# Sangluisme/PSgradientSDF

Measured on AMD Instinct MI355X. Metric: Gauss-Newton iterations/sec (full PS sweep), 256^3 grid x 50 frames, higher is better.
Workload: dtype f32

## Files before the change

psgradientsdf_amd/capi.py:

```python
from __future__ import annotations

import ctypes as C
import os

import numpy as np

ALBEDO, LIGHT, DIST, POSE, ALL = 1, 2, 4, 8, 15
SH1, SH2, LED = 0, 1, 2
L2, CAUCHY, HUBER, TUKEY, TRUNC_L2 = 0, 1, 2, 3, 4
R_DEPTH, R_NORMAL, R_ALBEDO, R_SHADING, R_RENDERED, R_RESIDUAL, R_VOXEL = 1, 2, 4, 8, 16, 32, 64
R_ALL = 127
_R_PLANES = [("depth", R_DEPTH, 1), ("normal", R_NORMAL, 3), ("albedo", R_ALBEDO, 3), ("shading", R_SHADING, 1),
             ("rendered", R_RENDERED, 3), ("residual", R_RESIDUAL, 3), ("voxel", R_VOXEL, 1)]

_HERE = os.path.dirname(os.path.abspath(__file__))
ENGINE_LIB = os.environ.get("PSGSDF_ENGINE_LIB") or os.path.join(_HERE, "csrc", "libpsgsdf.so")
ENGINE_LIB_DEV = os.path.join(_HERE, "csrc", "libpsgsdf_dev.so")


class GridDesc(C.Structure):
    _fields_ = [("dim", C.c_int32 * 3), ("voxel_size", C.c_float), ("shift", C.c_float * 3), ("truncation", C.c_float)]


class Settings(C.Structure):
# ... 806 lines not shown
                    cross_rank_ready=out[4] % 10, halo_pushes=out[4] // 10, cross_rank_solves=out[5], cross_rank_mem_kind=out[6], probe_stale=out[7] // 1000000, probe_timeouts=out[7] % 1000000)

    def debug_rare_rows(self):
        r = C.c_int64(); w = C.c_int64()
        self._check(self._fn("debug_rare_rows")(self.ctx, C.byref(r), C.byref(w)), "debug_rare_rows")
        return r.value, w.value

    def debug_frame_system(self, block):
        i = self.info()
        if block == LIGHT:
            n = i.light_stride; nb = 1 if self._settings.model == LED else i.n_frames
        else:
            n = 6; nb = i.n_frames
        H = np.empty((nb, n, n), np.float64); b = np.empty((nb, n), np.float64)
        self._check(self._fn("debug_frame_system")(self.ctx, C.c_int(block), H.ctypes.data_as(C.c_void_p), b.ctypes.data_as(C.c_void_p)), "debug_frame_system")
        return H, b

    def set_frame_solver(self, mode):
        self._check(self._fn("set_frame_solver")(self.ctx, C.c_int(mode)), "set_frame_solver")

    def frame_solver_stats(self, block):
        it = C.c_int32(); err = C.c_double(); ok = C.c_int32(); ap = C.c_int32()
        self._check(self._fn("get_frame_solver_stats")(self.ctx, C.c_int(block), C.byref(it), C.byref(err), C.byref(ok), C.byref(ap)), "get_frame_solver_stats")
        return {"cg_iters": it.value, "cg_error": err.value, "cg_converged": ok.value, "applied": ap.value}

    def debug_frame_cg(self, H, b, max_it=0):
        H = np.ascontiguousarray(H, np.float32); b = np.ascontiguousarray(b, np.float32)
        nb, n = b.shape
        x = np.empty((nb, n), np.float32); it = C.c_int32(); err = C.c_double(); ok = C.c_int32()
        self._check(self._fn("debug_frame_cg")(self.ctx, C.c_int(nb), C.c_int(n), H.ctypes.data_as(C.c_void_p), b.ctypes.data_as(C.c_void_p), x.ctypes.data_as(C.c_void_p),
                                               C.c_int(max_it), C.byref(it), C.byref(err), C.byref(ok)), "debug_frame_cg")
        return x, it.value, err.value, bool(ok.value)

    def debug_albedo_system(self):
        S = self.info().n_band
        H = np.empty((S, 3), np.float32); b = np.empty((S, 3), np.float32)
        self._check(self._fn("debug_albedo_system")(self.ctx, H.ctypes.data_as(C.c_void_p), b.ctypes.data_as(C.c_void_p)), "debug_albedo_system")
        return H, b


class CommXfer(C.Structure):
    _fields_ = [("ptr_dev", C.c_void_p), ("bytes", C.c_size_t), ("peer", C.c_int)]


ALLREDUCE_FN = C.CFUNCTYPE(C.c_int, C.c_void_p, C.c_void_p, C.c_int, C.c_void_p)
SENDRECV_FN = C.CFUNCTYPE(C.c_int, C.c_void_p, C.POINTER(CommXfer), C.c_int, C.POINTER(CommXfer), C.c_int, C.c_void_p)


class CommOps(C.Structure):
    _fields_ = [("user", C.c_void_p), ("allreduce_f64", ALLREDUCE_FN), ("sendrecv", SENDRECV_FN)]


def comm_unique_id() -> bytes:
    buf = (C.c_uint8 * 128)()
    f = engine_lib().psgsdf_comm_unique_id; f.restype = C.c_int
    rc = f(buf)
    if rc != 0:
        raise PsgsdfError(f"psgsdf_comm_unique_id failed rc={rc} (librccl could not be loaded?)")
    return bytes(buf)


def grid_of(sc) -> GridDesc:
    g = GridDesc()
    g.dim[:] = [int(x) for x in sc.dim]
    g.voxel_size = float(sc.voxel_size)
    g.shift[:] = [float(x) for x in sc.shift]
# ... 20 lines not shown
```

psgradientsdf_amd/csrc/api_debug.hip:

```cpp
#include "engine_internal.h"

using namespace psge;

extern "C" {
int psgsdf_set_profiling(psgsdf_ctx* c, int enabled) { if (!c) return PSGSDF_ERR_ARG; c->profiling = enabled != 0; return PSGSDF_OK; }
int psgsdf_reset_kernel_times(psgsdf_ctx* c) { if (!c) return PSGSDF_ERR_ARG; c->ktimes.clear(); c->watch_used = 0; return PSGSDF_OK; }
int psgsdf_watch_kernel(psgsdf_ctx* c, const char* name) {
    if (!c) return PSGSDF_ERR_ARG;
    hipStreamSynchronize(c->stream);
    std::string w = name ? name : ""; int every = 1;
    const size_t sl = w.find('/');
    if (sl != std::string::npos) { every = std::max(1, atoi(w.c_str() + sl + 1)); w.resize(sl); }
    c->watch = w; c->watch_every = every; c->watch_seen = 0; c->watch_used = 0;
    return PSGSDF_OK;
}
int psgsdf_kernel_times(psgsdf_ctx* c, const char** names, double* ms, int64_t* launches, int cap) {
    if (!c) return 0;
    if (c->watch_used) {
        hipStreamSynchronize(c->stream);
        KTime& k = c->ktimes[c->watch];
        for (size_t i = 0; i < c->watch_used; ++i) { float t = 0; if (hipEventElapsedTime(&t, c->watch_pool[i].first, c->watch_pool[i].second) == hipSuccess) { k.ms += t; k.n += 1; } }
        c->watch_used = 0;
    }
    int n = 0;
    for (auto& kv : c->ktimes) { if (n >= cap) break; names[n] = kv.first.c_str(); ms[n] = kv.second.ms; launches[n] = kv.second.n; ++n; }
    return n;
}

int psgsdf_debug_dist_system(psgsdf_ctx* c, float* diag, float* rhs, const float* x, float* y) {
    if (!c || !c->inited) return fail(c, PSGSDF_ERR_STATE, "init first");
    HIPCHK(c, hipSetDevice(c->device));
    SweepArgs a = make_args(c, c->reg_l != 0.f);
    launch_sweep_dist(a, c->stream);
// ... 131 lines not shown
int psgsdf_get_frame_solver_stats(psgsdf_ctx* c, int block, int32_t* iterations, double* error, int32_t* converged, int32_t* applied) {
    if (!c) return PSGSDF_ERR_ARG;
    if (block != PSGSDF_LIGHT && block != PSGSDF_POSE) return fail(c, PSGSDF_ERR_ARG, "block must be LIGHT or POSE");
    HIPCHK(c, hipSetDevice(c->device));
    const int kind = block == PSGSDF_POSE ? 1 : 0;
    psgsdf_step_stats st; memset(&st, 0, sizeof(st));
    if (int rc = read_frame_solver_stats(c, kind, &st)) return rc;
    if (iterations) *iterations = st.cg_iters;
    if (error) *error = st.cg_error;
    if (converged) *converged = st.cg_converged;
    if (applied) *applied = st.applied;
    return PSGSDF_OK;
}
int psgsdf_debug_frame_cg(psgsdf_ctx* c, int nb, int n, const float* H, const float* b, float* x, int max_it, int32_t* iterations, double* error, int32_t* converged) {
    if (!c || !H || !b || !x || nb <= 0) return fail(c, PSGSDF_ERR_ARG, "null argument");
    if ((n != 3 && n != 4 && n != 6 && n != 9) || (long long)nb * n > 2048) return fail(c, PSGSDF_ERR_UNSUPPORTED, "block size %d x %d blocks", n, nb);
    HIPCHK(c, hipSetDevice(c->device));
    float *dH = nullptr, *db = nullptr, *dx = nullptr; double* ds = nullptr;
    const size_t nH = (size_t)nb * n * n, nv = (size_t)nb * n;
    int rc = PSGSDF_OK;
    if (hipMalloc(&dH, sizeof(float) * nH) != hipSuccess || hipMalloc(&db, sizeof(float) * nv) != hipSuccess || hipMalloc(&dx, sizeof(float) * nv) != hipSuccess || hipMalloc(&ds, sizeof(double) * 4) != hipSuccess)
        rc = fail(c, PSGSDF_ERR_DEVICE, "out of device memory");
    double st[4] = {0, 0, 0, 0};
    if (!rc && (hipMemcpy(dH, H, sizeof(float) * nH, hipMemcpyHostToDevice) != hipSuccess || hipMemcpy(db, b, sizeof(float) * nv, hipMemcpyHostToDevice) != hipSuccess)) rc = fail(c, PSGSDF_ERR_DEVICE, "upload failed");
    if (!rc && launch_frames_eigen_raw(nb, n, dH, db, dx, ds, max_it, c->stream)) rc = fail(c, PSGSDF_ERR_UNSUPPORTED, "shape");
    if (!rc && (hipStreamSynchronize(c->stream) != hipSuccess || hipMemcpy(x, dx, sizeof(float) * nv, hipMemcpyDeviceToHost) != hipSuccess || hipMemcpy(st, ds, sizeof(st), hipMemcpyDeviceToHost) != hipSuccess))
        rc = fail(c, PSGSDF_ERR_DEVICE, "%s", hipGetErrorString(hipGetLastError()));
    hipFree(dH); hipFree(db); hipFree(dx); hipFree(ds);
    if (rc) return rc;
    if (iterations) *iterations = (int32_t)st[0];
    if (error) *error = st[1];
    if (converged) *converged = (int32_t)st[2];
    return PSGSDF_OK;
}
int psgsdf_debug_frame_system(psgsdf_ctx* c, int block, double* H, double* b) {
    if (!c || !c->inited || !H || !b) return fail(c, PSGSDF_ERR_STATE, "init first");
    HIPCHK(c, hipSetDevice(c->device));
    SweepArgs a = make_args(c, 0);
    const bool led = c->set.model == PSGSDF_LED;
    int n, nb, nh;
    int launched = 0;
    if (block == PSGSDF_LIGHT) { launched = launch_sweep_light(a, c->stream); n = led ? 3 : (c->set.model == PSGSDF_SH2 ? 9 : 4); nb = led ? 1 : c->F; nh = led ? 3 : n * (n + 1) / 2; }
    else if (block == PSGSDF_POSE) { launched = launch_sweep_pose(a, c->stream); n = 6; nb = c->F; nh = 21; }
    else return fail(c, PSGSDF_ERR_ARG, "block must be LIGHT or POSE");
    if (!launched) HIPCHK(c, hipMemsetAsync(c->acc_frame, 0, sizeof(double) * c->acc_frame_n, c->stream));
    std::vector<double> acc(c->acc_frame_n);
    HIPCHK(c, hipMemcpyAsync(acc.data(), c->acc_frame, sizeof(double) * c->acc_frame_n, hipMemcpyDeviceToHost, c->stream));
    HIPCHK(c, hipStreamSynchronize(c->stream));
    if (led && block == PSGSDF_LIGHT) {
        for (int i = 0; i < 9; ++i) H[i] = 0;
        for (int i = 0; i < 3; ++i) { b[i] = 0; for (int f = 0; f < c->F; ++f) { H[i * 3 + i] += acc[(size_t)f * kFrameRow + i]; b[i] += acc[(size_t)f * kFrameRow + 3 + i]; } }
        return PSGSDF_OK;
    }
    for (int k = 0; k < nb; ++k) {
        const double* A = acc.data() + (size_t)k * kFrameRow;
        double* Hk = H + (size_t)k * n * n; double* bk = b + (size_t)k * n;
        for (int i = 0; i < n * n; ++i) Hk[i] = 0;
        int q = 0;
        for (int i = 0; i < n; ++i) for (int j = i; j < n; ++j) { Hk[i * n + j] = A[q]; Hk[j * n + i] = A[q]; ++q; }
        for (int i = 0; i < n; ++i) bk[i] = A[nh + i];
    }
    return PSGSDF_OK;
}

int psgsdf_debug_albedo_system(psgsdf_ctx* c, float* H, float* b) {
    if (!c || !c->inited || !H || !b) return fail(c, PSGSDF_ERR_STATE, "init first");
// ... 68 lines not shown
```

psgradientsdf_amd/csrc/engine.h:

```cpp
#pragma once
#include <hip/hip_runtime.h>
#include <stdint.h>

namespace psg {

constexpr int kBlock = 256;
constexpr int kMaxFramesLds = 640;
constexpr int kNQ = 19;
constexpr int kNQCommon = 13;
constexpr int kMaxBasis = 9;

struct FrameP {
    float R[9];
    float t[3];
    float l[9];
    float pad[3];
};

struct Cam { float fx, fy, cx, cy; int W, H; };

struct GridP {
    int dim[3];
    long long nvox;
    float vs, vs_inv;
// ... 134 lines not shown
void launch_select_vis(const uint64_t* vis_seq, int wpv_seq, uint64_t* vis_key, int KW, const int* frame_idx, int F, long long nvox, hipStream_t s);
void launch_band_flags(const float* dist, const uint64_t* vis_key, int KW, float vs, long long nvox, int* flags, hipStream_t s);
void launch_band_scan(int* flags_inout_rowof, long long nvox, int* block_sums, int* d_total, hipStream_t s);
struct DenseView { float* dist; float* g[3]; float* weight; float* rho[3]; uint64_t* vis; int KW; int* row_of; };
void launch_band_fill(const DenseView& d, const GridP& grid, Band b, int* d_reach, hipStream_t s);
void launch_band_scatter(const DenseView& d, Band b, hipStream_t s);
void launch_derive(const SweepArgs& a, int update_grad, hipStream_t s);
constexpr int kObsChunk = 2048;
void launch_obs_count(const Band& b, int F, int row0, int row1, int* counts, hipStream_t s);
void launch_block_work(const Band& b, int row0, int row1, int* work, hipStream_t s);
void launch_obs_fill(const Band& b, int F, int row0, int row1, const int* offsets, hipStream_t s);
void launch_lower_bound(const int* lin, int S, int target, int* out, hipStream_t s);
struct SlotList { int n; int id[8]; };
void launch_sum_parts(const double* part, int PB, int nblk, const SlotList& slots, double* out, unsigned long long key, hipStream_t s, const XfTable* xf = nullptr, long long xf_epoch = 0);
void launch_frame_cols(const double* frame, int F, int col, double* out, unsigned long long key, hipStream_t s);
void launch_zero_f64(double* p, int n, hipStream_t s);
struct CopySegs { int n; unsigned off[16]; unsigned len[16]; unsigned long long key[16]; };
void launch_copy_segs(const double* src, double* dst, const CopySegs& segs, hipStream_t s);
void launch_marker(double* p, double v, hipStream_t s);
void launch_init_albedo(const SweepArgs& a, hipStream_t s);
void launch_led_light_init(const SweepArgs& a, hipStream_t s);
void launch_energy(const SweepArgs& a, hipStream_t s);
void launch_sweep_albedo(const SweepArgs& a, hipStream_t s);
void launch_apply_albedo(const SweepArgs& a, hipStream_t s);
void launch_restore_albedo(const SweepArgs& a, hipStream_t s);
int launch_sweep_light(const SweepArgs& a, hipStream_t s);
int launch_sweep_pose(const SweepArgs& a, hipStream_t s);
void launch_solve_light(const SweepArgs& a, FrameP* frames, float* led_light, double* e_out, unsigned long long e_key, float* undo, hipStream_t s);
void launch_restore_light(int F, FrameP* frames, float* led_light, const float* undo, hipStream_t s);
void launch_solve_pose(const SweepArgs& a, FrameP* frames, double* e_out, unsigned long long e_key, hipStream_t s);
bool frames_eigen_fits(int model, int F);
void launch_frames_eigen_light(const SweepArgs& a, FrameP* frames, float* led_light, double* e_out, unsigned long long e_key, float* undo, double* stats, hipStream_t s);
void launch_frames_eigen_pose(const SweepArgs& a, FrameP* frames, double* e_out, unsigned long long e_key, double* stats, hipStream_t s);
int launch_frames_eigen_raw(int nb, int n, const float* H, const float* b, float* x, double* stats, int max_it, hipStream_t s);
void launch_sweep_dist(const SweepArgs& a, hipStream_t s);
void launch_assemble(const SweepArgs& a, hipStream_t s);
void launch_cgf_init(const SweepArgs& a, double* fs, double* part, int G, hipStream_t s);
void launch_cgf_pass(const SweepArgs& a, double* fs, double* part, int G, int rows, int k, int kmax, double* mb, hipStream_t s, int ablate = 0);
void launch_cgf_sum(double* part, int G, int k, double* out, hipStream_t s);
constexpr int kSolveGranPlanes = 8;
constexpr int kSolveThreadsHost = 512, kSolveMaxBlocksHost = 256, kSolveMaxRowsHost = 4, kSolveMbSlots = 24;
int cgf_solve_max_blocks(int rows);
void launch_solve_windows(const Band& b, int row0, int row1, int G, int rows_per_wg, int* tab , int* max_total, hipStream_t s);
int cgf_solve_window_budget(int rows_per_wg);
int launch_cgf_solve(const SweepArgs& a, double* fs, double* gran, int G, int rows_per_wg, int kmax, double* mb, unsigned long long mb_key, int force_passes, hipStream_t s, const XrArgs* xr = nullptr);
void launch_areg_tables(const DenseView& d, const GridP& g, const SweepArgs& a, hipStream_t s);
void launch_areg_build(const SweepArgs& a, hipStream_t s);
void launch_areg_system(const SweepArgs& a, hipStream_t s);
void launch_areg_jx(const SweepArgs& a, const float* p, float* t, hipStream_t s);
void launch_areg_jt(const SweepArgs& a, const float* p, const float* t, float* q, hipStream_t s);
void launch_areg_cg_init(const SweepArgs& a, hipStream_t s);
void launch_areg_cg_iteration(const SweepArgs& a, int i, int nblk, float thr, hipStream_t s);
void launch_areg_cg_update(const SweepArgs& a, float alpha, hipStream_t s);
void launch_areg_cg_dir(const SweepArgs& a, float beta, hipStream_t s);
void launch_apply_albedo_delta(const SweepArgs& a, const float* delta, hipStream_t s);
void launch_matvec(const SweepArgs& a, const float* x, float* y, hipStream_t s);
void launch_apply_dist(const SweepArgs& a, hipStream_t s);
void launch_upsample(const DenseView& src, const DenseView& dst, const GridP& g_old, hipStream_t s);
void launch_fill_f32(float* p, float v, long long n, hipStream_t s);
void launch_normals(const float* depth, const float* cache, int W, int H, int r, double* tmp, float* out, hipStream_t s);
void launch_track(const DenseView& d, const GridP& g, const Cam& cam, const FrameP& fp, const float* depth, float z_min, float z_max, double* part, int nblk, int gdimz, int zown0, int zown1, hipStream_t s);
void launch_integrate(const DenseView& d, uint64_t* vis_seq, int wpv_seq, const GridP& g, const Cam& cam, const FrameP& fp,
                      const float* rgb, const float* depth, const float* normals, int counter, float z_min, float z_max, hipStream_t s);

constexpr int kRenderBrick = 8;
constexpr int kRenderTile = 8;
// ... 73 lines not shown
```

psgradientsdf_amd/csrc/sweeps.hip:

```cpp
#include "device_common.h"

#ifndef PSG_FM_PIPE
#define PSG_FM_PIPE 3
#endif
#ifndef PSG_POSE_WAVES
#define PSG_POSE_WAVES 1
#endif

namespace psg {

__global__ void __launch_bounds__(kBlock) k_init_albedo(SweepArgs a) {
#pragma clang fp contract(off)
    FrameP* sf = reinterpret_cast<FrameP*>(psg_dyn_smem);
    load_frames(sf, a.frames, a.F);
    const Band& b = a.b;
    int j = a.row0 + blockIdx.x * blockDim.x + threadIdx.x;
    if (j >= a.row1) return;
    const float4 p0 = b.vp[0][j];
    float xs[3] = {p0.x, p0.y, p0.z};
    int count = 0; float rho[3] = {0, 0, 0};
    FOR_EACH_VISIBLE_FRAME(b, j, a.F, f) {
        Proj pr = project(xs, frame_at(sf, f), a.cam);
        if (!pr.ok) continue;
        float I[3];
        sample<false>(a.im, f, a.cam, pr.m, pr.n, I, nullptr, nullptr);
        rho[0] += I[0]; rho[1] += I[1]; rho[2] += I[2]; count++;
    }
    if (count) {
#pragma unroll
        for (int k = 0; k < 3; ++k) set_rho(b, j, k, rho[k] / (float)count);
    }
}
void launch_init_albedo(const SweepArgs& a, hipStream_t s) {
    if (a.row1 > a.row0) hipLaunchKernelGGL(k_init_albedo, dim3((a.row1 - a.row0 + kBlock - 1) / kBlock), dim3(kBlock), a.F * sizeof(FrameP), s, a);
}

template <int MODEL, int LOSS, int IMG, bool LED_INIT = false>
__global__ void __launch_bounds__(kBlock) k_energy(SweepArgs a) {
    { __shared__ double fred[kBlock / 64]; fold_pending(a, fred); }
// ... 133 lines not shown
    if (j >= a.row1) return;
#pragma unroll
    for (int ch = 0; ch < 3; ++ch) set_rho(b, j, ch, b.aH[(size_t)ch * b.Spad + j]);
}
void launch_restore_albedo(const SweepArgs& a, hipStream_t s) {
    if (a.row1 > a.row0) hipLaunchKernelGGL(k_restore_albedo, dim3((a.row1 - a.row0 + kBlock - 1) / kBlock), dim3(kBlock), 0, s, a);
}
void launch_apply_albedo(const SweepArgs& a, hipStream_t s) {
    if (a.row1 > a.row0) hipLaunchKernelGGL(k_apply_albedo, dim3((a.row1 - a.row0 + kBlock - 1) / kBlock), dim3(kBlock), 0, s, a);
}

static int fm_rows(const SweepArgs& a, int slots_per_cu) {
    if (const char* e = getenv("PSGSDF_FM_ROWS")) { int v = atoi(e); if (v >= 4 && v <= 64) return v; }
    const long long total = a.b.obs_ptr_total > 0 ? a.b.obs_ptr_total : (long long)a.b.obs_max * a.F;
    const long long slots = 256LL * slots_per_cu;
    long long r = (total + (long long)(0.92 * slots) * kBlock - 1) / ((long long)(0.92 * slots) * kBlock);
    return (int)std::min<long long>(std::max<long long>(r, 4), 64);
}

template <int N> __device__ void solve_spd(const double* Hin, const double* bin, double* x);

__device__ __forceinline__ double ldrow(const double* p) { return __hip_atomic_load(p, __ATOMIC_RELAXED, __HIP_MEMORY_SCOPE_AGENT); }
template <int NB>
__device__ __forceinline__ void frame_solve_light_sh(FrameP* frames, int f, const double* acc, float* undo) {
    constexpr int NH = NB * (NB + 1) / 2;
    if (undo) for (int i = 0; i < 9; ++i) undo[f * 9 + i] = frames[f].l[i];
    double Hd[NB * NB], bd[NB], xd[NB];
    int q = 0;
    for (int i = 0; i < NB; ++i) for (int k = i; k < NB; ++k) { double v = (double)(float)ldrow(acc + q++); Hd[i * NB + k] = v; Hd[k * NB + i] = v; }
    for (int i = 0; i < NB; ++i) bd[i] = (double)(float)ldrow(acc + NH + i);
    solve_spd<NB>(Hd, bd, xd);
    for (int i = 0; i < NB; ++i) frames[f].l[i] -= (float)xd[i];
}
__device__ __forceinline__ void frame_solve_pose(const SweepArgs& a, FrameP* frames, int f, const double* acc) {
    double Hd[36], bd[6], xd[6];
    int q = 0;
    for (int i = 0; i < 6; ++i) for (int k = i; k < 6; ++k) {
        float v = (float)ldrow(acc + q++);
        if (i == k && a.damping != 0.0f) v += a.damping * v;
        Hd[i * 6 + k] = (double)v; Hd[k * 6 + i] = (double)v;
    }
    for (int i = 0; i < 6; ++i) bd[i] = (double)(float)ldrow(acc + 21 + i);
    solve_spd<6>(Hd, bd, xd);
    float xi[6];
    for (int i = 0; i < 6; ++i) xi[i] = (float)xd[i];
    pose_update(frames, f, xi);
}

template <int NV, int KIND, int MODEL>
__device__ __forceinline__ void frame_tail(const SweepArgs& a, double* lds, bool solve_all) {
    if (solve_all) {
        for (int ff = threadIdx.x; ff < a.F; ff += blockDim.x) {
            const double* row = a.acc.frame + (size_t)ff * kFrameRow;
            if (KIND == 0) { if (!ModelTraits<MODEL>::LED) frame_solve_light_sh<ModelTraits<MODEL>::NB == 3 ? 4 : ModelTraits<MODEL>::NB>(a.fm_frames, ff, row, a.fm_undo); }
            else frame_solve_pose(a, a.fm_frames, ff, row);
        }
        __syncthreads();
    }
    if (KIND == 0 && ModelTraits<MODEL>::LED) {
        constexpr int NHL = 3;
        __shared__ float s_dl[3];
        if (a.fm_undo) {
            for (int i = threadIdx.x; i < a.F * 9; i += blockDim.x) a.fm_undo[i] = a.fm_frames[i / 9].l[i % 9];
            if (threadIdx.x < 3) a.fm_undo[a.F * 9 + threadIdx.x] = a.fm_led_light[threadIdx.x];
        }
        __shared__ double srow[6 * kMaxFramesLds];
        for (int i = threadIdx.x; i < 6 * a.F; i += blockDim.x) { const int ff = i / 6, c6 = i % 6; srow[c6 * kMaxFramesLds + ff] = __hip_atomic_load(a.acc.frame + (size_t)ff * kFrameRow + (c6 < 3 ? c6 : NHL + c6 - 3), __ATOMIC_RELAXED, __HIP_MEMORY_SCOPE_AGENT); }
        __syncthreads();
        if (threadIdx.x < 3) {
            const int ch = threadIdx.x;
            double hs = 0, bs = 0;
            for (int ff = 0; ff < a.F; ++ff) { hs += srow[ch * kMaxFramesLds + ff]; bs += srow[(3 + ch) * kMaxFramesLds + ff]; }
            float h = (float)hs; const float bb = (float)bs;
            if (a.damping != 0.0f) h += a.damping * h;
            double Hd[1] = {(double)h}, bd[1] = {(double)bb}, xd[1];
            solve_spd<1>(Hd, bd, xd);
            s_dl[ch] = (float)xd[0];
        }
        __syncthreads();
        for (int ff = threadIdx.x; ff < a.F; ff += blockDim.x) {
#pragma unroll
            for (int ch = 0; ch < 3; ++ch) { const float nl = a.fm_frames[ff].l[ch] - s_dl[ch]; a.fm_frames[ff].l[ch] = nl; if (ff == 0) a.fm_led_light[ch] = nl; }
        }
    }
    if (a.fm_e_out) {
        constexpr int col_e = NV - 2;
        double e = 0, n = 0;
        for (int ff = threadIdx.x; ff < a.F; ff += blockDim.x) {
            e += __hip_atomic_load(a.acc.frame + (size_t)ff * kFrameRow + col_e, __ATOMIC_RELAXED, __HIP_MEMORY_SCOPE_AGENT);
            n += __hip_atomic_load(a.acc.frame + (size_t)ff * kFrameRow + col_e + 1, __ATOMIC_RELAXED, __HIP_MEMORY_SCOPE_AGENT);
        }
        e = wave_sum(e); n = wave_sum(n);
        const int lane = threadIdx.x & 63, w = threadIdx.x >> 6;
        __syncthreads();
        if (lane == 0) { lds[2 * w] = e; lds[2 * w + 1] = n; }
        __syncthreads();
        if (threadIdx.x == 0) { double te = 0, tn = 0; for (int i = 0; i < (int)(blockDim.x >> 6); ++i) { te += lds[2 * i]; tn += lds[2 * i + 1]; } mbox_put(a.fm_e_out, 2, 0, te, a.fm_e_key); mbox_put(a.fm_e_out, 2, 1, tn, a.fm_e_key); mbox_commit(a.fm_e_key); }
    }
}

template <int NV, int KIND, int MODEL>
__device__ __forceinline__ void frame_rows_publish(const SweepArgs& a, int cx, int f, double* lds ) {
    __shared__ int s_last;
    double* dst = a.acc.fpart + ((size_t)f * a.acc.fcap + cx) * kFrameRow;
    if (threadIdx.x < NV) {
        double s = 0;
        for (int i = 0; i < kBlock / 64; ++i) s += lds[i * NV + threadIdx.x];
        __hip_atomic_store(dst + threadIdx.x, s, __ATOMIC_RELAXED, __HIP_MEMORY_SCOPE_AGENT);
    }
    if (threadIdx.x < 64) {
        asm volatile("s_waitcnt vmcnt(0)" ::: "memory");
        if (threadIdx.x == 0) s_last = __hip_atomic_fetch_add(a.acc.fdone + f, 1, __ATOMIC_RELAXED, __HIP_MEMORY_SCOPE_AGENT) == (int)gridDim.x - 1;
    }
    __syncthreads();
    if (!s_last) return;
    if (threadIdx.x == 0) __hip_atomic_store(a.acc.fdone + f, 0, __ATOMIC_RELAXED, __HIP_MEMORY_SCOPE_AGENT);
    const bool solve = a.fm_solve != 0;
    if (threadIdx.x < NV) {
        const double* p = a.acc.fpart + (size_t)f * a.acc.fcap * kFrameRow + threadIdx.x;
        double s = 0;
        for (int c = 0; c < (int)gridDim.x; c += 16) {
            double v[16];
#pragma unroll
            for (int j = 0; j < 16; ++j) v[j] = c + j < (int)gridDim.x ? __hip_atomic_load(p + (size_t)(c + j) * kFrameRow, __ATOMIC_RELAXED, __HIP_MEMORY_SCOPE_AGENT) : 0.0;
#pragma unroll
            for (int j = 0; j < 16; ++j) s += v[j];
        }
        if (solve && a.xf) {
            const XfTable& t = *a.xf;
            const int Rk = t.n_ranks, buf = (int)(a.xf_epoch & 1);
            const long long slot = ((long long)buf * Rk + t.rank) * t.F + f;
            for (int r = 0; r < Rk; ++r) store8_system(t.region[r] + t.pay + slot * kFrameRow + threadIdx.x, s);
            asm volatile("s_waitcnt vmcnt(0)" ::: "memory");
            if (threadIdx.x == 0) for (int r = 0; r < Rk; ++r) __hip_atomic_store(t.region[r] + t.flg + slot, (double)a.xf_epoch, __ATOMIC_RELAXED, __HIP_MEMORY_SCOPE_SYSTEM);
        }
        else if (solve) { __hip_atomic_store(a.acc.frame + (size_t)f * kFrameRow + threadIdx.x, s, __ATOMIC_RELAXED, __HIP_MEMORY_SCOPE_AGENT); lds[threadIdx.x] = s; }
        else a.acc.frame[(size_t)f * kFrameRow + threadIdx.x] = s;
    }
    if (!solve) return;
    if (a.xf) return;
    __syncthreads();
    if (threadIdx.x == 0) {
        if (KIND == 0) { if (!ModelTraits<MODEL>::LED) frame_solve_light_sh<ModelTraits<MODEL>::NB == 3 ? 4 : ModelTraits<MODEL>::NB>(a.fm_frames, f, lds, a.fm_undo); }
        else frame_solve_pose(a, a.fm_frames, f, lds);
    }
    if (threadIdx.x < 64) {
        asm volatile("s_waitcnt vmcnt(0)" ::: "memory");
        if (threadIdx.x == 0) s_last = __hip_atomic_fetch_add(a.acc.fdone + a.F, 1, __ATOMIC_RELAXED, __HIP_MEMORY_SCOPE_AGENT) == (int)gridDim.y - 1;
    }
    __syncthreads();
    if (!s_last) return;
    if (threadIdx.x == 0) __hip_atomic_store(a.acc.fdone + a.F, 0, __ATOMIC_RELAXED, __HIP_MEMORY_SCOPE_AGENT);
    frame_tail<NV, KIND, MODEL>(a, lds, false);
}

constexpr int kGatherFrames = 16;
template <int NV, int KIND, int MODEL>
__global__ void __launch_bounds__(kBlock) k_frame_gather(SweepArgs a) {
    __shared__ double lds[(kBlock / 64) * NV > 2 * (kBlock / 64) ? (kBlock / 64) * NV : 2 * (kBlock / 64)];
    __shared__ unsigned char s_late[kGatherFrames];
    __shared__ int s_last;
    const XfTable& t = *a.xf;
    const int Rk = t.n_ranks, buf = (int)(a.xf_epoch & 1);
    const double tag = (double)a.xf_epoch;
    double* const mine = t.region[t.rank];
    const int f0 = blockIdx.x * kGatherFrames, nf = min(kGatherFrames, a.F - f0);
    if (threadIdx.x < kGatherFrames) s_late[threadIdx.x] = 0;
    __syncthreads();
    for (int q = threadIdx.x; q < nf * Rk; q += blockDim.x) {
        const int ff = f0 + q / Rk, r = q - (q / Rk) * Rk;
        const double* fp = mine + t.flg + ((long long)buf * Rk + r) * t.F + ff;
        int spins = 0; bool late = false;
        while (__hip_atomic_load(fp, __ATOMIC_RELAXED, __HIP_MEMORY_SCOPE_SYSTEM) != tag) { __builtin_amdgcn_s_sleep(2); if (++spins > t.spin_max) { late = true; break; } }
        if (late) {
            s_late[ff - f0] = 1;
            __hip_atomic_store(mine + kXrLate, tag, __ATOMIC_RELAXED, __HIP_MEMORY_SCOPE_SYSTEM);
            __hip_atomic_store(mine + kXrLate + 3, (double)(r * 1000 + ff), __ATOMIC_RELAXED, __HIP_MEMORY_SCOPE_SYSTEM);
        }
    }
    __builtin_amdgcn_fence(__ATOMIC_ACQUIRE, "");
    __syncthreads();
    for (int i = threadIdx.x; i < nf * NV; i += blockDim.x) {
        const int fl = i / NV, l = i - fl * NV, ff = f0 + fl;
        const double* p0 = mine + t.pay + ((long long)buf * Rk * t.F + ff) * kFrameRow + l;
        double tot = 0.0;
        for (int r0 = 0; r0 < Rk; r0 += 8) {
// ... 97 lines not shown
        }
#endif
        acc[NH + NB] += (obs_acc_t)l; acc[NH + NB + 1] += 1;
    };
    const int e0 = beg + cx * (kBlock * rows) + threadIdx.x;
    if constexpr (IMG >= 0 && !(PSG_STRICT & 4) && (PSG_FM_PIPE & 1)) {
        fm_for_each_obs<IMG>(b, fp, a.cam, img, e0, end, rows, [&](const ObsPend<IMG>& P) {
            float I[3];
            taps_colour<IMG, false>(img, a.cam, P.ts, P.pr.m, P.pr.n, P.pr.m, P.pr.n, I, nullptr, nullptr);
            accumulate(P.v, P.pr, I);
            return true;
        }, [&](const Vox&, const Proj&) {});
    } else {
    int e = e0;
    int j_cur = e < end ? b.obs_rows[e] : -1;
    int j_nxt = (rows > 1 && e + kBlock < end) ? b.obs_rows[e + kBlock] : -1;
    Vox vn;
    if (j_cur >= 0) load_vox(b, j_cur, vn);
    for (int it = 0; it < rows && j_cur >= 0; ++it, e += kBlock) {
        const Vox v = vn;
        const int j_nn = (it + 2 < rows && e + 2 * kBlock < end) ? b.obs_rows[e + 2 * kBlock] : -1;
        if (j_nxt >= 0) load_vox(b, j_nxt, vn);
        j_cur = j_nxt; j_nxt = j_nn;
        Proj pr = project(v.xs, fp, a.cam);
        if (!pr.ok) continue;
        float I[3];
        sample<false, IMG>(img, 0, a.cam, pr.m, pr.n, I, nullptr, nullptr);
        accumulate(v, pr, I);
    }
    }
    const int w = threadIdx.x >> 6;
    wave_sums_to<NV>(acc, lds + w * NV);
    __syncthreads();
    frame_rows_publish<NV, 0, MODEL>(a, cx, f, lds);
}
int launch_sweep_light(const SweepArgs& a, hipStream_t s) {
    if (a.b.S <= 0 || a.F <= 0 || a.b.obs_max <= 0) return 0;
    const int rows = fm_rows(a, a.model == 1 ? 3 : ((PSG_FM_PIPE & 1) ? 4 : 5));
    const int chunk = kBlock * rows;
    dim3 g((a.b.obs_max + chunk - 1) / chunk, a.F), bl(kBlock);
    PSG_LAUNCH_SWEEP(k_sweep_light, a, true, g, bl, 0, s, a, rows);
    if (a.xf && a.fm_solve) launch_frame_gather<0>(a, s);
    return (int)g.x;
}

template <int MODEL, int LOSS, int IMG>
__global__ void __launch_bounds__(kBlock, PSG_POSE_WAVES) k_sweep_pose(SweepArgs a, int rows) {
    { __shared__ double fred[kBlock / 64]; fold_pending(a, fred); }
    constexpr int NB = ModelTraits<MODEL>::NB;
    constexpr bool LED = ModelTraits<MODEL>::LED;
    constexpr int NV = 21 + 6 + 2;
    __shared__ FrameP sfp;
    __shared__ double lds[(kBlock / 64) * NV];
    int cx, f; fm_ids(a, cx, f);
    if (threadIdx.x < (int)(sizeof(FrameP) / 4)) ((float*)&sfp)[threadIdx.x] = ((const float*)(a.frames + f))[threadIdx.x];
    __syncthreads();
    const Band& b = a.b;
    const FrameP& fp = sfp;
    ImgSrc img = a.im;
    if (img.u8) img.u8 += (size_t)f * a.cam.H * a.cam.W; else img.f32 += (size_t)f * a.cam.H * a.cam.W * 3;
    img.idx32 = true;
    obs_acc_t acc[NV];
#pragma unroll
    for (int k = 0; k < NV; ++k) acc[k] = 0;
    const int beg = b.obs_ptr[f], end = b.obs_ptr[f + 1];
    auto accumulate = [&](const Vox& v, const Proj& pr, const ProjJ& pj, const float* I, const float* gu, const float* gv) {
// ... 97 lines not shown
            const ProjJ pj = project_jac(P.pr, a.cam);
            float I[3], gu[3], gv[3];
            if (!taps_colour<IMG, true>(img, a.cam, P.ts, P.pr.m, P.pr.n, pj.mj, pj.nj, I, gu, gv)) return false;
            accumulate(P.v, P.pr, pj, I, gu, gv);
            return true;
        }, [&](const Vox& v, const Proj& pr) {
            const ProjJ pj = project_jac(pr, a.cam);
            float I[3], gu[3], gv[3];
            sample<true, IMG>(img, 0, a.cam, pr.m, pr.n, pj.mj, pj.nj, I, gu, gv);
            accumulate(v, pr, pj, I, gu, gv);
        });
    } else {
    int e = e0;
    int j_cur = e < end ? b.obs_rows[e] : -1;
    int j_nxt = (rows > 1 && e + kBlock < end) ? b.obs_rows[e + kBlock] : -1;
    Vox vn;
    if (j_cur >= 0) load_vox(b, j_cur, vn);
    for (int it = 0; it < rows && j_cur >= 0; ++it, e += kBlock) {
        const Vox v = vn;
        const int j_nn = (it + 2 < rows && e + 2 * kBlock < end) ? b.obs_rows[e + 2 * kBlock] : -1;
        if (j_nxt >= 0) load_vox(b, j_nxt, vn);
        j_cur = j_nxt; j_nxt = j_nn;
        Proj pr = project(v.xs, fp, a.cam);
        if (!pr.ok) continue;
        float I[3], gu[3], gv[3];
        const ProjJ pj = project_jac(pr, a.cam);
        sample<true, IMG>(img, 0, a.cam, pr.m, pr.n, pj.mj, pj.nj, I, gu, gv);
        accumulate(v, pr, pj, I, gu, gv);
    }
    }
    const int w = threadIdx.x >> 6;
    wave_sums_to<NV>(acc, lds + w * NV);
    __syncthreads();
    frame_rows_publish<NV, 1, MODEL>(a, cx, f, lds);
}
int launch_sweep_pose(const SweepArgs& a, hipStream_t s) {
    if (a.b.S <= 0 || a.F <= 0 || a.b.obs_max <= 0) return 0;
    const int rows = fm_rows(a, ((PSG_FM_PIPE & 2) && PSG_POSE_WAVES < 4) ? 3 : 4);
    const int chunk = kBlock * rows;
    dim3 g((a.b.obs_max + chunk - 1) / chunk, a.F), bl(kBlock);
    PSG_LAUNCH_SWEEP(k_sweep_pose, a, true, g, bl, 0, s, a, rows);
    if (a.xf && a.fm_solve) launch_frame_gather<1>(a, s);
    return (int)g.x;
}

template <int N>
__device__ void solve_spd(const double* Hin, const double* bin, double* x) {
    double L[N * N], D[N], y[N];
    double scale = 0;
    for (int i = 0; i < N; ++i) scale = fmax(scale, fabs(Hin[i * N + i]));
    const double tiny = scale * 1e-12;
    for (int i = 0; i < N * N; ++i) L[i] = 0;
    for (int j = 0; j < N; ++j) {
        double d = Hin[j * N + j];
        for (int k = 0; k < j; ++k) d -= L[j * N + k] * L[j * N + k] * D[k];
        D[j] = d; L[j * N + j] = 1.0;
        for (int i = j + 1; i < N; ++i) {
            double s = Hin[i * N + j];
            for (int k = 0; k < j; ++k) s -= L[i * N + k] * L[j * N + k] * D[k];
            L[i * N + j] = (d > tiny) ? s / d : 0.0;
        }
    }
    for (int i = 0; i < N; ++i) { double s = bin[i]; for (int k = 0; k < i; ++k) s -= L[i * N + k] * y[k]; y[i] = s; }
    for (int i = 0; i < N; ++i) y[i] = (D[i] > tiny) ? y[i] / D[i] : 0.0;
    for (int i = N - 1; i >= 0; --i) { double s = y[i]; for (int k = i + 1; k < N; ++k) s -= L[k * N + i] * x[k]; x[i] = s; }
}
// ... 44 lines not shown
            dl[ch] = (float)xd[0];
        }
        for (int f = threadIdx.x; f < a.F; f += blockDim.x) {
#pragma unroll
            for (int ch = 0; ch < 3; ++ch) { const float nl = frames[f].l[ch] - dl[ch]; frames[f].l[ch] = nl; if (f == 0) led_light[ch] = nl; }
        }
    } else {
        for (int f = threadIdx.x; f < a.F; f += blockDim.x) frame_solve_light_sh<NB>(frames, f, a.acc.frame + (size_t)f * kFrameRow, nullptr);
    }
    frame_rows_finish(a, NH + NB, e_out, e_key, red);
}
__global__ void __launch_bounds__(kBlock) k_restore_light(int F, FrameP* frames, float* led_light, const float* undo) {
    for (int i = threadIdx.x; i < F * 9; i += blockDim.x) frames[i / 9].l[i % 9] = undo[i];
    if (threadIdx.x < 3) led_light[threadIdx.x] = undo[F * 9 + threadIdx.x];
}
void launch_restore_light(int F, FrameP* frames, float* led_light, const float* undo, hipStream_t s) { if (F > 0) hipLaunchKernelGGL(k_restore_light, dim3(1), dim3(kBlock), 0, s, F, frames, led_light, undo); }
void launch_solve_light(const SweepArgs& a, FrameP* frames, float* led_light, double* e_out, unsigned long long e_key, float* undo, hipStream_t s) {
    if (a.F <= 0) return;
    dim3 g(1), bl(kBlock);
    if (a.model == 0) hipLaunchKernelGGL((k_solve_light<0>), g, bl, 0, s, a, frames, led_light, e_out, e_key, undo);
    else if (a.model == 1) hipLaunchKernelGGL((k_solve_light<1>), g, bl, 0, s, a, frames, led_light, e_out, e_key, undo);
    else hipLaunchKernelGGL((k_solve_light<2>), g, bl, 0, s, a, frames, led_light, e_out, e_key, undo);
}

__global__ void __launch_bounds__(kBlock) k_solve_pose(SweepArgs a, FrameP* frames, double* e_out, unsigned long long e_key) {
    __shared__ double red[2 * kBlock / 64];
    for (int f = threadIdx.x; f < a.F; f += blockDim.x) frame_solve_pose(a, frames, f, a.acc.frame + (size_t)f * kFrameRow);
    frame_rows_finish(a, 27, e_out, e_key, red);
}
void launch_solve_pose(const SweepArgs& a, FrameP* frames, double* e_out, unsigned long long e_key, hipStream_t s) {
    if (a.F > 0) hipLaunchKernelGGL(k_solve_pose, dim3(1), dim3(kBlock), 0, s, a, frames, e_out, e_key);
}

}
```

Measured before the change: 3180.

## Parallelize frame-tail solves across a wave and overlap last-frame reduction

In the fused frame tail, each per-frame light or pose LDLT solve is now spread across the 64 lanes of a wave using readlane broadcasts, where before one thread ran a serial factorization. The last-frame counter increment now happens before the solve, so the final workgroup's energy reduction runs on a second wave alongside the solve instead of after it. Stage-timestamp instrumentation and debug entry points are added for checking the lane solver against the scalar one. The risks are different floating-point results and extra register pressure from the lane solver.

```diff
diff --git a/include/psgsdf_debug.h b/include/psgsdf_debug.h
--- /dev/null
+++ b/include/psgsdf_debug.h
@@ -0,0 +1,14 @@
+#ifndef PSGSDF_DEBUG_H
+#define PSGSDF_DEBUG_H
+#include "psgsdf.h"
+#ifdef __cplusplus
+extern "C" {
+#endif
+
+int psgsdf_debug_frame_ldlt(psgsdf_ctx* ctx, int n_blocks, int n, const double* H, const double* b, double* x_scalar, double* x_lanes);
+int psgsdf_debug_frame_tail_stages(psgsdf_ctx* ctx, int block, int reps, double us[6]);
+
+#ifdef __cplusplus
+}
+#endif
+#endif
diff --git a/psgradientsdf_amd/capi.py b/psgradientsdf_amd/capi.py
--- a/psgradientsdf_amd/capi.py
+++ b/psgradientsdf_amd/capi.py
@@ -862,6 +862,19 @@
                                                C.c_int(max_it), C.byref(it), C.byref(err), C.byref(ok)), "debug_frame_cg")
         return x, it.value, err.value, bool(ok.value)
 
+    def debug_frame_ldlt(self, H, b):
+        H = np.ascontiguousarray(H, np.float64); b = np.ascontiguousarray(b, np.float64)
+        nb, n = b.shape
+        xs = np.empty((nb, n), np.float64); xl = np.empty((nb, n), np.float64)
+        self._check(self._fn("debug_frame_ldlt")(self.ctx, C.c_int(nb), C.c_int(n), H.ctypes.data_as(C.c_void_p), b.ctypes.data_as(C.c_void_p), xs.ctypes.data_as(C.c_void_p),
+                                                 xl.ctypes.data_as(C.c_void_p)), "debug_frame_ldlt")
+        return xs, xl
+
+    def debug_frame_tail_stages(self, block, reps=40):
+        us = (C.c_double * 6)()
+        self._check(self._fn("debug_frame_tail_stages")(self.ctx, C.c_int(block), C.c_int(reps), us), "debug_frame_tail_stages")
+        return [x for x in us]
+
     def debug_albedo_system(self):
         S = self.info().n_band
         H = np.empty((S, 3), np.float32); b = np.empty((S, 3), np.float32)
diff --git a/psgradientsdf_amd/csrc/api_debug.hip b/psgradientsdf_amd/csrc/api_debug.hip
--- a/psgradientsdf_amd/csrc/api_debug.hip
+++ b/psgradientsdf_amd/csrc/api_debug.hip
@@ -1,4 +1,5 @@
 #include "engine_internal.h"
+#include "../../include/psgsdf_debug.h"
 
 using namespace psge;
 
@@ -196,6 +197,47 @@
     if (error) *error = st[1];
     if (converged) *converged = (int32_t)st[2];
     return PSGSDF_OK;
+}
+int psgsdf_debug_frame_ldlt(psgsdf_ctx* c, int nb, int n, const double* H, const double* b, double* x_scalar, double* x_lanes) {
+    if (!c || !H || !b || !x_scalar || !x_lanes || nb <= 0) return fail(c, PSGSDF_ERR_ARG, "null argument");
+    if (n != 1 && n != 4 && n != 6 && n != 9) return fail(c, PSGSDF_ERR_UNSUPPORTED, "block size %d", n);
+    HIPCHK(c, hipSetDevice(c->device));
+    double *dH = nullptr, *db = nullptr, *dx = nullptr;
+    const size_t nH = (size_t)nb * n * n, nv = (size_t)nb * n;
+    int rc = PSGSDF_OK;
+    if (hipMalloc(&dH, sizeof(double) * nH) != hipSuccess || hipMalloc(&db, sizeof(double) * nv) != hipSuccess || hipMalloc(&dx, sizeof(double) * 2 * nv) != hipSuccess) rc = fail(c, PSGSDF_ERR_DEVICE, "out of device memory");
+    if (!rc && (hipMemcpy(dH, H, sizeof(double) * nH, hipMemcpyHostToDevice) != hipSuccess || hipMemcpy(db, b, sizeof(double) * nv, hipMemcpyHostToDevice) != hipSuccess)) rc = fail(c, PSGSDF_ERR_DEVICE, "upload failed");
+    if (!rc && launch_debug_ldlt(nb, n, dH, db, dx, dx + nv, c->stream)) rc = fail(c, PSGSDF_ERR_UNSUPPORTED, "shape");
+    if (!rc && (hipStreamSynchronize(c->stream) != hipSuccess || hipMemcpy(x_scalar, dx, sizeof(double) * nv, hipMemcpyDeviceToHost) != hipSuccess || hipMemcpy(x_lanes, dx + nv, sizeof(double) * nv, hipMemcpyDeviceToHost) != hipSuccess))
+        rc = fail(c, PSGSDF_ERR_DEVICE, "%s", hipGetErrorString(hipGetLastError()));
+    hipFree(dH); hipFree(db); hipFree(dx);
+    return rc;
+}
+int psgsdf_debug_frame_tail_stages(psgsdf_ctx* c, int block, int reps, double* us) {
+    if (!c || !c->inited || !us || reps < 1) return fail(c, PSGSDF_ERR_STATE, "init first");
+    if (block != PSGSDF_LIGHT && block != PSGSDF_POSE) return fail(c, PSGSDF_ERR_ARG, "block must be LIGHT or POSE");
+    if (c->n_ranks > 1 || (block == PSGSDF_LIGHT && c->set.model == PSGSDF_LED)) return fail(c, PSGSDF_ERR_UNSUPPORTED, "stage stamps: one rank, per-frame solves");
+    HIPCHK(c, hipSetDevice(c->device));
+    if (tail_stamps_reset(c->stream) == 1) return fail(c, PSGSDF_ERR_UNSUPPORTED, "this library's sweeps carry no stage stamps (the development library's do)");
+    { int rc = flush(c); if (rc) return rc; }
+    FrameP* fr = nullptr; float* undo = nullptr; double* slot = nullptr; double* slot_dev = nullptr;
+    int rc = PSGSDF_OK;
+    if (hipMalloc(&fr, sizeof(FrameP) * c->F) != hipSuccess || hipMalloc(&undo, sizeof(float) * (9 * (size_t)c->F + 3)) != hipSuccess || hipHostMalloc(&slot, sizeof(double) * 8, hipHostMallocMapped) != hipSuccess
+        || hipHostGetDevicePointer((void**)&slot_dev, slot, 0) != hipSuccess) rc = fail(c, PSGSDF_ERR_DEVICE, "out of memory");
+    const int kind = block == PSGSDF_POSE ? 1 : 0;
+    for (int j = 0; j < 6; ++j) us[j] = 0;
+    for (int r = 0; r < reps + 1 && !rc; ++r) {
+        SweepArgs a = make_args(c, 0);
+        a.fm_solve = 1; a.fm_frames = fr; a.fm_led_light = c->led_light; a.fm_e_out = slot_dev; a.fm_e_key = 0x5ca1ab1e00ull + (unsigned long long)r; a.fm_undo = kind == 0 ? undo : nullptr;
+        if (hipMemcpyAsync(fr, c->frames, sizeof(FrameP) * c->F, hipMemcpyDeviceToDevice, c->stream) != hipSuccess || tail_stamps_reset(c->stream)) { rc = fail(c, PSGSDF_ERR_DEVICE, "stage stamps: set-up"); break; }
+        const int launched = kind ? launch_sweep_pose(a, c->stream) : launch_sweep_light(a, c->stream);
+        if (!launched) { rc = fail(c, PSGSDF_ERR_STATE, "no observations"); break; }
+        unsigned long long t[6];
+        if (tail_stamps_read(kind, t, c->stream)) { rc = fail(c, PSGSDF_ERR_DEVICE, "%s", hipGetErrorString(hipGetLastError())); break; }
+        if (r) for (int j = 0; j < 6; ++j) us[j] += ((double)t[j] - (double)t[0]) * 0.01 / reps;
+    }
+    hipFree(fr); hipFree(undo); if (slot) hipHostFree(slot);
+    return rc;
 }
 int psgsdf_debug_frame_system(psgsdf_ctx* c, int block, double* H, double* b) {
     if (!c || !c->inited || !H || !b) return fail(c, PSGSDF_ERR_STATE, "init first");
diff --git a/psgradientsdf_amd/csrc/engine.h b/psgradientsdf_amd/csrc/engine.h
--- a/psgradientsdf_amd/csrc/engine.h
+++ b/psgradientsdf_amd/csrc/engine.h
@@ -190,6 +190,9 @@
 bool frames_eigen_fits(int model, int F);
 void launch_frames_eigen_light(const SweepArgs& a, FrameP* frames, float* led_light, double* e_out, unsigned long long e_key, float* undo, double* stats, hipStream_t s);
 void launch_frames_eigen_pose(const SweepArgs& a, FrameP* frames, double* e_out, unsigned long long e_key, double* stats, hipStream_t s);
+int launch_debug_ldlt(int nb, int n, const double* H, const double* b, double* x_scalar, double* x_lanes, hipStream_t s);
+int tail_stamps_reset(hipStream_t s);
+int tail_stamps_read(int kind, unsigned long long* latest , hipStream_t s);
 int launch_frames_eigen_raw(int nb, int n, const float* H, const float* b, float* x, double* stats, int max_it, hipStream_t s);
 void launch_sweep_dist(const SweepArgs& a, hipStream_t s);
 void launch_assemble(const SweepArgs& a, hipStream_t s);
diff --git a/psgradientsdf_amd/csrc/sweeps.hip b/psgradientsdf_amd/csrc/sweeps.hip
--- a/psgradientsdf_amd/csrc/sweeps.hip
+++ b/psgradientsdf_amd/csrc/sweeps.hip
@@ -5,6 +5,15 @@
 #endif
 #ifndef PSG_POSE_WAVES
 #define PSG_POSE_WAVES 1
+#endif
+#ifndef PSG_FM_TAIL
+#define PSG_FM_TAIL 3
+#endif
+#ifdef PSG_FM_TAIL_STAMPS
+namespace psg { constexpr int kTailStampWgs = 4096; __device__ unsigned long long g_tail_ts[2][6][kTailStampWgs]; }
+#define TAIL_STAMP(KIND, j) do { const unsigned wg_ = blockIdx.y * gridDim.x + blockIdx.x; if (wg_ < (unsigned)kTailStampWgs) g_tail_ts[KIND][j][wg_] = wall_clock64(); } while (0)
+#else
+#define TAIL_STAMP(KIND, j) do { } while (0)
 #endif
 
 namespace psg {
@@ -204,12 +213,12 @@
     solve_spd<NB>(Hd, bd, xd);
     for (int i = 0; i < NB; ++i) frames[f].l[i] -= (float)xd[i];
 }
+__device__ __forceinline__ float pose_h_elem(const SweepArgs& a, double r, bool diag) { float v = (float)r; if (diag && a.damping != 0.0f) v += a.damping * v; return v; }
 __device__ __forceinline__ void frame_solve_pose(const SweepArgs& a, FrameP* frames, int f, const double* acc) {
     double Hd[36], bd[6], xd[6];
     int q = 0;
     for (int i = 0; i < 6; ++i) for (int k = i; k < 6; ++k) {
-        float v = (float)ldrow(acc + q++);
-        if (i == k && a.damping != 0.0f) v += a.damping * v;
+        const float v = pose_h_elem(a, ldrow(acc + q++), i == k);
         Hd[i * 6 + k] = (double)v; Hd[k * 6 + i] = (double)v;
     }
     for (int i = 0; i < 6; ++i) bd[i] = (double)(float)ldrow(acc + 21 + i);
@@ -217,6 +226,70 @@
     float xi[6];
     for (int i = 0; i < 6; ++i) xi[i] = (float)xd[i];
     pose_update(frames, f, xi);
+}
+
+__device__ __forceinline__ double lane_get(double v, int l) { return __hiloint2double(__builtin_amdgcn_readlane(__double2hiint(v), l), __builtin_amdgcn_readlane(__double2loint(v), l)); }
+template <int N>
+__device__ __forceinline__ void solve_spd_lanes(const double (&Hrow)[N], double bi, double (&x)[N]) {
+#pragma clang fp contract(off)
+    const int lane = threadIdx.x & 63;
+    double scale = 0;
+#pragma unroll
+    for (int i = 0; i < N; ++i) scale = fmax(scale, fabs(lane_get(Hrow[i], i)));
+    const double tiny = scale * 1e-12;
+    double L[N], D[N], dmine = 0;
+#pragma unroll
+    for (int j = 0; j < N; ++j) {
+        double v = Hrow[j];
+#pragma unroll
+        for (int k = 0; k < j; ++k) v = __builtin_fma(-(L[k] * lane_get(L[k], j)), D[k], v);
+        const double d = lane_get(v, j);
+        D[j] = d;
+        if (lane == j) dmine = d;
+        L[j] = 0.0;
+        if (j + 1 < N) { const double q = (d > tiny) ? v / d : 0.0; L[j] = lane > j ? q : 0.0; }
+    }
+    double s = bi;
+#pragma unroll
+    for (int k = 0; k + 1 < N; ++k) { const double yk = lane_get(s, k); if (lane > k) s = __builtin_fma(-L[k], yk, s); }
+    const double y = (dmine > tiny) ? s / dmine : 0.0;
+#pragma unroll
+    for (int i = N - 1; i >= 0; --i) {
+        double t = lane_get(y, i);
+#pragma unroll
+        for (int k = i + 1; k < N; ++k) t = __builtin_fma(-lane_get(L[i], k), x[k], t);
+        x[i] = t;
+    }
+}
+template <int N> __device__ __forceinline__ int tri_at(int i, int k) { const int lo = min(i, k), hi = max(i, k); return lo * N - (lo * (lo - 1)) / 2 + (hi - lo); }
+template <int NB>
+__device__ __forceinline__ void frame_solve_light_sh_lanes(FrameP* frames, int f, const double* row, float* undo) {
+    constexpr int NH = NB * (NB + 1) / 2;
+    const int lane = threadIdx.x & 63, li = min(lane, NB - 1);
+    if (undo && lane < 9) undo[f * 9 + lane] = frames[f].l[lane];
+    const float l0 = frames[f].l[li];
+    double Hrow[NB], xd[NB];
+#pragma unroll
+    for (int k = 0; k < NB; ++k) Hrow[k] = (double)(float)row[tri_at<NB>(li, k)];
+    solve_spd_lanes<NB>(Hrow, (double)(float)row[NH + li], xd);
+    double xm = 0;
+#pragma unroll
+    for (int k = 0; k < NB; ++k) xm = lane == k ? xd[k] : xm;
+    if (lane < NB) frames[f].l[lane] = l0 - (float)xm;
+}
+__device__ __forceinline__ void frame_solve_pose_lanes(const SweepArgs& a, FrameP* frames, int f, const double* row) {
+    const int lane = threadIdx.x & 63, li = min(lane, 5);
+    double Hrow[6], xd[6];
+#pragma unroll
+    for (int k = 0; k < 6; ++k) {
+        Hrow[k] = (double)pose_h_elem(a, row[tri_at<6>(li, k)], li == k);
+    }
+    solve_spd_lanes<6>(Hrow, (double)(float)row[21 + li], xd);
+    if (lane == 0) {
+        float xi[6];
+        for (int i = 0; i < 6; ++i) xi[i] = (float)xd[i];
+        pose_update(frames, f, xi);
+    }
 }
 
 template <int NV, int KIND, int MODEL>
@@ -282,7 +355,7 @@
     }
     if (threadIdx.x < 64) {
         asm volatile("s_waitcnt vmcnt(0)" ::: "memory");
-        if (threadIdx.x == 0) s_last = __hip_atomic_fetch_add(a.acc.fdone + f, 1, __ATOMIC_RELAXED, __HIP_MEMORY_SCOPE_AGENT) == (int)gridDim.x - 1;
+        if (threadIdx.x == 0) { s_last = __hip_atomic_fetch_add(a.acc.fdone + f, 1, __ATOMIC_RELAXED, __HIP_MEMORY_SCOPE_AGENT) == (int)gridDim.x - 1; TAIL_STAMP(KIND, 1); }
     }
     __syncthreads();
     if (!s_last) return;
@@ -311,19 +384,56 @@
     }
     if (!solve) return;
     if (a.xf) return;
-    __syncthreads();
-    if (threadIdx.x == 0) {
-        if (KIND == 0) { if (!ModelTraits<MODEL>::LED) frame_solve_light_sh<ModelTraits<MODEL>::NB == 3 ? 4 : ModelTraits<MODEL>::NB>(a.fm_frames, f, lds, a.fm_undo); }
-        else frame_solve_pose(a, a.fm_frames, f, lds);
-    }
+    constexpr bool kLedLight = KIND == 0 && ModelTraits<MODEL>::LED;
+    constexpr int NBS = ModelTraits<MODEL>::NB == 3 ? 4 : ModelTraits<MODEL>::NB;
+    if (threadIdx.x == 0) TAIL_STAMP(KIND, 2);
+    auto solve_frame = [&]() {
+        if (kLedLight) return;
+        if (PSG_FM_TAIL & 2) { if (KIND == 0) frame_solve_light_sh_lanes<NBS>(a.fm_frames, f, lds, a.fm_undo); else frame_solve_pose_lanes(a, a.fm_frames, f, lds); }
+        else if (threadIdx.x == 0) { if (KIND == 0) frame_solve_light_sh<NBS>(a.fm_frames, f, lds, a.fm_undo); else frame_solve_pose(a, a.fm_frames, f, lds); }
+        if (threadIdx.x == 0) TAIL_STAMP(KIND, 3);
+    };
+    if ((PSG_FM_TAIL & 1) && !kLedLight) {
+        __shared__ int s_last_frame;
+        if (threadIdx.x < 64) {
+            asm volatile("s_waitcnt vmcnt(0)" ::: "memory");
+            if (threadIdx.x == 0) { s_last_frame = __hip_atomic_fetch_add(a.acc.fdone + a.F, 1, __ATOMIC_RELAXED, __HIP_MEMORY_SCOPE_AGENT) == (int)gridDim.y - 1; TAIL_STAMP(KIND, 4); }
+        }
+        __syncthreads();
+        if (threadIdx.x < 64) solve_frame();
+        else if (threadIdx.x < 128 && s_last_frame) {
+            const int lane = threadIdx.x & 63;
+            if (lane == 0) __hip_atomic_store(a.acc.fdone + a.F, 0, __ATOMIC_RELAXED, __HIP_MEMORY_SCOPE_AGENT);
+            if (a.fm_e_out) {
+                constexpr int col_e = NV - 2;
+                double e[kBlock / 64], n[kBlock / 64];
+#pragma unroll
+                for (int w = 0; w < kBlock / 64; ++w) {
+                    e[w] = 0; n[w] = 0;
+                    for (int ff = w * 64 + lane; ff < a.F; ff += kBlock) {
+                        e[w] += __hip_atomic_load(a.acc.frame + (size_t)ff * kFrameRow + col_e, __ATOMIC_RELAXED, __HIP_MEMORY_SCOPE_AGENT);
+                        n[w] += __hip_atomic_load(a.acc.frame + (size_t)ff * kFrameRow + col_e + 1, __ATOMIC_RELAXED, __HIP_MEMORY_SCOPE_AGENT);
+                    }
+                }
+                double te = 0, tn = 0;
+#pragma unroll
+                for (int w = 0; w < kBlock / 64; ++w) { te += wave_sum(e[w]); tn += wave_sum(n[w]); }
+                if (lane == 0) { mbox_put(a.fm_e_out, 2, 0, te, a.fm_e_key); mbox_put(a.fm_e_out, 2, 1, tn, a.fm_e_key); mbox_commit(a.fm_e_key); TAIL_STAMP(KIND, 5); }
+            }
+        }
+        return;
+    }
+    __syncthreads();
+    if (threadIdx.x < 64) solve_frame();
     if (threadIdx.x < 64) {
         asm volatile("s_waitcnt vmcnt(0)" ::: "memory");
-        if (threadIdx.x == 0) s_last = __hip_atomic_fetch_add(a.acc.fdone + a.F, 1, __ATOMIC_RELAXED, __HIP_MEMORY_SCOPE_AGENT) == (int)gridDim.y - 1;
+        if (threadIdx.x == 0) { s_last = __hip_atomic_fetch_add(a.acc.fdone + a.F, 1, __ATOMIC_RELAXED, __HIP_MEMORY_SCOPE_AGENT) == (int)gridDim.y - 1; TAIL_STAMP(KIND, 4); }
     }
     __syncthreads();
     if (!s_last) return;
     if (threadIdx.x == 0) __hip_atomic_store(a.acc.fdone + a.F, 0, __ATOMIC_RELAXED, __HIP_MEMORY_SCOPE_AGENT);
     frame_tail<NV, KIND, MODEL>(a, lds, false);
+    if (threadIdx.x == 0) TAIL_STAMP(KIND, 5);
 }
 
 constexpr int kGatherFrames = 16;
@@ -487,6 +597,7 @@
     const int w = threadIdx.x >> 6;
     wave_sums_to<NV>(acc, lds + w * NV);
     __syncthreads();
+    if (threadIdx.x == 0) TAIL_STAMP(0, 0);
     frame_rows_publish<NV, 0, MODEL>(a, cx, f, lds);
 }
 int launch_sweep_light(const SweepArgs& a, hipStream_t s) {
@@ -650,6 +761,7 @@
     const int w = threadIdx.x >> 6;
     wave_sums_to<NV>(acc, lds + w * NV);
     __syncthreads();
+    if (threadIdx.x == 0) TAIL_STAMP(1, 0);
     frame_rows_publish<NV, 1, MODEL>(a, cx, f, lds);
 }
 int launch_sweep_pose(const SweepArgs& a, hipStream_t s) {
@@ -760,4 +872,56 @@
     if (a.F > 0) hipLaunchKernelGGL(k_solve_pose, dim3(1), dim3(kBlock), 0, s, a, frames, e_out, e_key);
 }
 
-}
+template <int N>
+__global__ void __launch_bounds__(64) k_debug_ldlt(const double* H, const double* b, double* x_scalar, double* x_lanes) {
+    const double* Hb = H + (size_t)blockIdx.x * N * N; const double* bb = b + (size_t)blockIdx.x * N;
+    const int lane = threadIdx.x, li = min(lane, N - 1);
+    if (lane == 0) {
+        double Hd[N * N], bd[N], xd[N];
+        for (int i = 0; i < N * N; ++i) Hd[i] = Hb[i];
+        for (int i = 0; i < N; ++i) bd[i] = bb[i];
+        solve_spd<N>(Hd, bd, xd);
+        for (int i = 0; i < N; ++i) x_scalar[(size_t)blockIdx.x * N + i] = xd[i];
+    }
+    double Hrow[N], xl[N];
+#pragma unroll
+    for (int k = 0; k < N; ++k) Hrow[k] = Hb[li * N + k];
+    solve_spd_lanes<N>(Hrow, bb[li], xl);
+    double xm = 0;
+#pragma unroll
+    for (int k = 0; k < N; ++k) xm = lane == k ? xl[k] : xm;
+    if (lane < N) x_lanes[(size_t)blockIdx.x * N + lane] = xm;
+}
+int launch_debug_ldlt(int nb, int n, const double* H, const double* b, double* x_scalar, double* x_lanes, hipStream_t s) {
+    if (nb <= 0) return 0;
+    const dim3 g(nb), bl(64);
+    if (n == 1) hipLaunchKernelGGL((k_debug_ldlt<1>), g, bl, 0, s, H, b, x_scalar, x_lanes);
+    else if (n == 4) hipLaunchKernelGGL((k_debug_ldlt<4>), g, bl, 0, s, H, b, x_scalar, x_lanes);
+    else if (n == 6) hipLaunchKernelGGL((k_debug_ldlt<6>), g, bl, 0, s, H, b, x_scalar, x_lanes);
+    else if (n == 9) hipLaunchKernelGGL((k_debug_ldlt<9>), g, bl, 0, s, H, b, x_scalar, x_lanes);
+    else return 1;
+    return 0;
+}
+int tail_stamps_reset(hipStream_t s) {
+#ifdef PSG_FM_TAIL_STAMPS
+    void* p = nullptr;
+    if (hipGetSymbolAddress(&p, HIP_SYMBOL(g_tail_ts)) != hipSuccess) return 2;
+    return hipMemsetAsync(p, 0, sizeof(unsigned long long) * 2 * 6 * kTailStampWgs, s) == hipSuccess ? 0 : 2;
+#else
+    return 1;
+#endif
+}
+int tail_stamps_read(int kind, unsigned long long* latest , hipStream_t s) {
+#ifdef PSG_FM_TAIL_STAMPS
+    void* p = nullptr;
+    if (kind < 0 || kind > 1 || hipGetSymbolAddress(&p, HIP_SYMBOL(g_tail_ts)) != hipSuccess) return 2;
+    std::vector<unsigned long long> h((size_t)6 * kTailStampWgs);
+    if (hipMemcpyAsync(h.data(), (const unsigned long long*)p + (size_t)kind * 6 * kTailStampWgs, sizeof(unsigned long long) * h.size(), hipMemcpyDeviceToHost, s) != hipSuccess || hipStreamSynchronize(s) != hipSuccess) return 2;
+    for (int j = 0; j < 6; ++j) { latest[j] = 0; for (int w = 0; w < kTailStampWgs; ++w) latest[j] = std::max(latest[j], h[(size_t)j * kTailStampWgs + w]); }
+    return 0;
+#else
+    return 1;
+#endif
+}
+
+}
```

Result: no change. 3205, median of 6 (+0.8%).
